# DylanAuty/ObjCAViT

Measured on AMD Instinct MI355X. Metric: images/sec (640x480, bs=16) forward depth inference, 3 batches of 16 in flight per GPU; AbsRel vs CPU ref, higher is better.
Workload: dtype f32 (fp16 / bf16 split contractions)

## Files before the change

### include/objcavit_hip.h

```cpp
#ifndef OBJCAVIT_HIP_H
#define OBJCAVIT_HIP_H

#include <stddef.h>
#include <stdint.h>

#ifdef __cplusplus
extern "C" {
#endif

typedef void* ocv_stream_t;

#define OCV_ABI_VERSION 5
int ocv_abi_version(void);
const char* ocv_last_error(void);

int ocv_range_flag_set(unsigned* flag);
int ocv_range_flag_take_fwd(unsigned* flag, unsigned* out, ocv_stream_t stream);
int ocv_attention_set_fp32_range(int on);
int ocv_attention_set_dispatch(int form);

#define OCV_ACT_NONE 0
#define OCV_ACT_RELU 1
#define OCV_ACT_LEAKY_RELU 2
#define OCV_ACT_SILU 3
// ... 92 lines not shown
                              void* workspace, size_t workspace_bytes, ocv_stream_t stream);

int ocv_pixel_dot_fwd(const float* feat, int channels_last, const float* queries, long q_bs, int q_ld, float* ram,
                      int B, int C, int Q, int P, ocv_stream_t stream);

size_t ocv_bin_head_workspace_bytes(int B, int n_bins, int C);
int ocv_bin_head_fold_fwd(const float* queries, long q_bs, int q_ld, const float* Wout, float* Wf, int B, int C, int Q,
                          int n_bins, ocv_stream_t stream);
int ocv_bin_head_folded_fwd(const float* feat, int channels_last, const float* Wf, const float* bout,
                            const float* centers, float* depth, int B, int C, int n_bins, int P, ocv_stream_t stream);
size_t ocv_bin_head_partials_bytes(int B, int P);
int ocv_bin_head_folded_ws_fwd(const float* feat, int channels_last, const float* Wf, const float* bout, const float* centers,
                               float* depth, int B, int C, int n_bins, int P, void* partials, size_t partials_bytes,
                               ocv_stream_t stream);
int ocv_bin_head_fwd(const float* feat, int channels_last, const float* queries, long q_bs, int q_ld, const float* Wout,
                     const float* bout, const float* centers, float* depth, int B, int C, int Q, int n_bins, int P,
                     void* workspace, size_t workspace_bytes, ocv_stream_t stream);
size_t ocv_bin_head_stats_partials_bytes(int B, int P);
int ocv_bin_head_folded_stats_fwd(const float* feat, int channels_last, const float* Wf, const float* bout, const float* centers,
                                  float* depth, int B, int C, int n_bins, int P, void* partials, size_t partials_bytes, float* var,
                                  float* pmax, ocv_stream_t stream);

int ocv_conv3x3_few_channels_fwd(const float* x, long stride_b, long stride_c, long stride_y, long stride_x, const float* w_taps,
                                 float* y, int B, int C, int H, int W, int Cout, ocv_stream_t stream);

int ocv_depthwise_conv_fwd(const float* in, const float* w, const float* bias, float* out, int B, int C, int H, int W,
                           int k, int stride, int pad_t, int pad_l, int Ho, int Wo, int act, ocv_stream_t stream);

int ocv_pointwise_conv_nhwc_fwd(const float* x, const float* gate, int rows_per_image, const float* W,
                                const float* bias, const float* residual, float* y, long M, int Cin, int Cout, int act,
                                ocv_stream_t stream);

size_t ocv_pointwise_packed_weight_elems(int Cin, int Cout);
int ocv_pointwise_split_set_dispatch(int family, int a, int b);
int ocv_pointwise_conv_nhwc_split_fwd(const float* x, const float* gate, int rows_per_image, const void* w_packed,
                                      const float* bias, const float* residual, float* y, long M, int Cin, int Cout,
                                      int act, ocv_stream_t stream);
int ocv_pointwise_conv_nhwc_split_hl_fwd(const float* x, const float* gate, int rows_per_image, const void* w_packed,
                                         const float* bias, const float* residual, float* y, void* y_hl, long M, int Cin,
                                         int Cout, int act, ocv_stream_t stream);
size_t ocv_pointwise_split_workspace_bytes(long M, int Cin, int Cout);
int ocv_pointwise_conv_nhwc_split_ws_fwd(const float* x, const float* gate, int rows_per_image, const void* w_packed,
                                         const float* bias, const float* residual, float* y, void* y_hl, long M, int Cin, int Cout,
                                         int act, void* workspace, size_t workspace_bytes, ocv_stream_t stream);
int ocv_pointwise_hl_set_dispatch(int rt, int tn);
int ocv_pointwise_hl_fwd(const void* x_hl, int Cin, const void* w_packed, long w_image_elems, int rows_per_image,
                         const float* bias, const float* residual, float* y, void* y_hl, long M, int Cout, int act,
                         ocv_stream_t stream);
int ocv_stem_conv_fwd(const float* x, const float* w, const float* bias, float* y, int B, int Cin, int H, int W, int Cout,
                      int k, int stride, int pad_t, int pad_l, int Ho, int Wo, int act, ocv_stream_t stream);
int ocv_depthwise_conv_nhwc_fwd(const float* in, const float* w, const float* bias, float* out, int B, int C, int H,
                                int W, int k, int stride, int pad_t, int pad_l, int Ho, int Wo, int act,
                                ocv_stream_t stream);
int ocv_depthwise_sum_tiles(int B, int C, int Ho, int Wo, int k, int stride);
int ocv_depthwise_conv_nhwc_sum_fwd(const float* in, const float* w, const float* bias, float* out, float* part, int B,
                                    int C, int H, int W, int k, int stride, int pad_t, int pad_l, int Ho, int Wo,
                                    ocv_stream_t stream);
int ocv_se_gate_partials_fwd(const float* part, int tiles, long pixels_per_image, const float* w1, const float* b1,
                             const float* w2t, const float* b2, float* gate, float* hidden_ws, int B, int C, int R,
                             ocv_stream_t stream);
int ocv_depthwise_conv_nhwc_sum_hl_fwd(const float* in, const float* w, const float* bias, float* out, void* out_hl, float* part,
                                       int B, int C, int H, int W, int k, int stride, int pad_t, int pad_l, int Ho, int Wo,
                                       ocv_stream_t stream);
int ocv_se_gate_weights_fwd(const float* part, int tiles, long pixels_per_image, const float* w1, const float* b1,
                            const float* w2t, const float* b2, const float* W, void* w_packed, long w_image_elems, float* gate,
                            float* hidden_ws, int B, int C, int R, int N, ocv_stream_t stream);


size_t ocv_channel_mean_workspace_bytes(int B, int C, long P);
int ocv_channel_mean_nhwc_fwd(const float* x, float* out, int B, int C, long P, void* workspace, size_t workspace_bytes,
                              ocv_stream_t stream);

int ocv_se_gate_fwd(const float* mean, const float* w1, const float* b1, const float* w2t, const float* b2, float* gate,
                    float* hidden_ws, int B, int C, int R, ocv_stream_t stream);

int ocv_conv_nhwc_fwd(const float* x1, int C1, const float* x2, int C2, const void* w_hi, const void* w_lo,
                      const float* bias, const float* residual, float* y, int B, int H, int W, int Cout, int ksize,
                      int act, ocv_stream_t stream);
int ocv_conv_nhwc_exact_fwd(const float* x1, int C1, const float* x2, int C2, const float* w_tap_major, const float* bias,
                            const float* residual, float* y, int B, int H, int W, int Cout, int ksize, int act,
                            ocv_stream_t stream);
int ocv_conv3x3_nhwc_strided_fwd(const float* x, int Cin, const void* w_hi, const void* w_lo, const float* bias,
                                 const float* residual, float* y, int B, int H, int W, int Cout, int stride, int pad_t,
                                 int pad_l, int Ho, int Wo, int act, ocv_stream_t stream);

int ocv_mbconv_expand_dw_tiles(int Ho, int Wo, int k, int stride);
int ocv_mbconv_expand_dw_fwd(const float* x, const void* w_packed, const float* bias_expand, const float* w_dw,
                             const float* bias_dw, float* y, float* part, int B, int H, int W, int Cin, int mid, int k,
                             int stride, int pad_t, int pad_l, int Ho, int Wo, ocv_stream_t stream);

size_t ocv_split_act_elems(int B, int H, int W, int C);

int ocv_conv_nhwc_split_fwd(const void* x_hl, int Cin, const void* w_hi, const void* w_lo, const float* bias,
                            const float* residual, float* y, void* y_hl, int B, int H, int W, int Cout, int ksize,
                            int act, ocv_stream_t stream);
size_t ocv_conv_nhwc_split_workspace_bytes(int B, int H, int W, int Cin, int Cout, int ksize);
int ocv_conv_nhwc_split_ws_fwd(const void* x_hl, int Cin, const void* w_hi, const void* w_lo, const float* bias,
                               const float* residual, float* y, void* y_hl, int B, int H, int W, int Cout, int ksize,
                               int act, void* workspace, size_t workspace_bytes, ocv_stream_t stream);
int ocv_conv_nhwc_split_x_fwd(const void* x_hl, int Cin, const void* w_hi, const void* w_lo, const float* oscale, int f16,
                              const float* bias, const float* residual, float* y, void* y_hl, int B, int H, int W, int Cout,
                              int ksize, int act, void* workspace, size_t workspace_bytes, ocv_stream_t stream);

int ocv_conv3x3_packed_taps_k(int Cin);
int ocv_conv3x3_split_packed_taps_fwd(const void* x_hl, int Cin, const void* w_hi, const void* w_lo, const float* oscale, int f16,
                                      const float* bias, const float* residual, float* y, void* y_hl, int B, int H, int W, int Cout,
// ... 84 lines not shown
```

### objcavit_amd/_lib.py

```python
from __future__ import annotations

import ctypes as C
import os
from typing import Optional

_HERE = os.path.dirname(os.path.abspath(__file__))
LIB_PATH = os.environ.get("OCV_LIB_PATH") or os.path.join(_HERE, "lib", "libobjcavit_hip.so")

_f32p = C.c_void_p
_u8p = C.c_void_p
_stream = C.c_void_p
ABI_VERSION = 5


class EncoderLayerParams(C.Structure):
    _fields_ = [("struct_size", C.c_size_t)] + [(n, C.c_void_p) for n in (
        "in_proj_w", "in_proj_b", "out_proj_w", "out_proj_b", "norm1_w", "norm1_b",
        "linear1_w", "linear1_b", "linear2_w", "linear2_b", "norm2_w", "norm2_b",
        "in_proj_p3", "out_proj_p3", "linear1_p3", "linear2_p3",
        "in_proj_h2", "out_proj_h2", "linear1_h2", "linear2_h2")]

    def __init__(self, *a, **kw):
        super().__init__(*a, **kw)
        self.struct_size = C.sizeof(EncoderLayerParams)
# ... 27 lines not shown
    "ocv_ffn_residual_layernorm_fwd": (C.c_int, [_f32p] * 7 + [C.c_float, _u8p, _f32p, C.c_int, C.c_int, C.c_int, _stream]),
    "ocv_split3_packed_elems": (C.c_size_t, [C.c_int, C.c_int]),
    "ocv_pack_split3_fwd": (C.c_int, [_f32p, C.c_int, C.c_int, C.c_int, C.c_void_p, _stream]),
    "ocv_linear_split3_fwd": (C.c_int, [_f32p, C.c_int, C.c_void_p, _f32p, _f32p, C.c_int, C.c_int, C.c_int, C.c_int, C.c_int, _stream]),
    "ocv_linear_residual_layernorm_split3_fwd": (C.c_int, [_f32p, C.c_int, C.c_void_p, _f32p, _f32p, C.c_int, _f32p, _f32p, C.c_float,
                                                           _u8p, _f32p, C.c_int, C.c_int, C.c_int, C.c_int, _stream]),
    "ocv_ffn_split3_workspace_bytes": (C.c_size_t, [C.c_int, C.c_int]),
    "ocv_ffn_residual_layernorm_split3_fwd": (C.c_int, [_f32p, C.c_void_p, _f32p, C.c_void_p, _f32p, _f32p, _f32p, C.c_float, _u8p, _f32p,
                                                        C.c_int, C.c_int, C.c_int, C.c_void_p, C.c_size_t, _stream]),
    "ocv_layer_tail_split3_fwd": (C.c_int, [_f32p, _f32p, C.POINTER(EncoderLayerParams), C.c_void_p, _f32p, C.c_float, _u8p, _f32p, _f32p,
                                            C.c_int, C.c_int, C.c_int, _stream]),
    "ocv_layer_tail_h2_fwd": (C.c_int, [_f32p, _f32p, C.POINTER(EncoderLayerParams), C.c_void_p, _f32p, C.c_float, _u8p, _f32p, _f32p,
                                            C.c_int, C.c_int, C.c_int, _stream]),
    "ocv_layer_tail_h2_groups": (C.c_int, [C.c_int, C.c_int]),
    "ocv_layer_tail_h2_workspace_bytes": (C.c_size_t, [C.c_int, C.c_int]),
    "ocv_layer_tail_h2_ws_fwd": (C.c_int, [_f32p, _f32p, C.POINTER(EncoderLayerParams), C.c_void_p, _f32p, C.c_float, _u8p, _f32p, _f32p,
                                           C.c_int, C.c_int, C.c_int, C.c_void_p, C.c_size_t, _stream]),
    "ocv_encoder_stack_workspace_bytes": (C.c_size_t, [C.c_int, C.c_int, C.c_int]),
    "ocv_encoder_stack_fwd": (C.c_int, [_f32p, C.POINTER(EncoderLayerParams), C.c_int, _u8p, C.c_int, _f32p, C.c_int, C.c_int, C.c_int,
                                        C.c_int, C.c_int, C.c_float, C.c_void_p, C.c_size_t, _stream]),
    "ocv_encoder_layer_workspace_bytes": (C.c_size_t, [C.c_int, C.c_int, C.c_int, C.c_int]),
    "ocv_encoder_layer_fwd": (C.c_int, [_f32p, C.POINTER(EncoderLayerParams), _u8p, C.c_int, _f32p, C.c_int, C.c_int,
                                        C.c_int, C.c_int, C.c_int, C.c_float, C.c_void_p, C.c_size_t, _stream]),
    "ocv_pointwise_conv_nhwc_split_hl_fwd": (C.c_int, [_f32p, _f32p, C.c_int, C.c_void_p, _f32p, _f32p, _f32p, C.c_void_p, C.c_long, C.c_int,
                                                       C.c_int, C.c_int, _stream]),
    "ocv_pointwise_split_workspace_bytes": (C.c_size_t, [C.c_long, C.c_int, C.c_int]),
    "ocv_pointwise_conv_nhwc_split_ws_fwd": (C.c_int, [_f32p, _f32p, C.c_int, C.c_void_p, _f32p, _f32p, _f32p, C.c_void_p, C.c_long, C.c_int,
                                                       C.c_int, C.c_int, C.c_void_p, C.c_size_t, _stream]),
    "ocv_pointwise_hl_set_dispatch": (C.c_int, [C.c_int, C.c_int]),
    "ocv_pointwise_hl_fwd": (C.c_int, [C.c_void_p, C.c_int, C.c_void_p, C.c_long, C.c_int, _f32p, _f32p, _f32p, C.c_void_p, C.c_long,
                                       C.c_int, C.c_int, _stream]),
    "ocv_depthwise_conv_nhwc_sum_hl_fwd": (C.c_int, [_f32p, _f32p, _f32p, _f32p, C.c_void_p, _f32p] + [C.c_int] * 10 + [_stream]),
    "ocv_se_gate_weights_fwd": (C.c_int, [_f32p, C.c_int, C.c_long, _f32p, _f32p, _f32p, _f32p, _f32p, C.c_void_p, C.c_long, _f32p,
                                          _f32p, C.c_int, C.c_int, C.c_int, C.c_int, _stream]),
    "ocv_patch_embed_workspace_bytes": (C.c_size_t, [C.c_int, C.c_int, C.c_int, C.c_int, C.c_int]),
    "ocv_patch_embed_split_workspace_bytes": (C.c_size_t, [C.c_int, C.c_int, C.c_int, C.c_int, C.c_int]),
    "ocv_patch_embed_split_fwd": (C.c_int, [C.c_void_p, C.c_int, C.c_void_p, C.c_void_p, _f32p, C.c_int, _f32p, _f32p, C.c_long, _f32p, C.c_int,
                                            C.c_int, C.c_int, C.c_int, C.c_void_p, C.c_size_t, _stream]),
    "ocv_patch_embed_fwd": (C.c_int, [_f32p, C.c_int, _f32p, _f32p, _f32p, C.c_long, _f32p, C.c_int, C.c_int, C.c_int, C.c_int,
                                      C.c_int, C.c_void_p, C.c_size_t, _stream]),
    "ocv_pixel_dot_fwd": (C.c_int, [_f32p, C.c_int, _f32p, C.c_long, C.c_int, _f32p, C.c_int, C.c_int, C.c_int, C.c_int, _stream]),
    "ocv_bin_head_workspace_bytes": (C.c_size_t, [C.c_int, C.c_int, C.c_int]),
    "ocv_bin_head_fold_fwd": (C.c_int, [_f32p, C.c_long, C.c_int, _f32p, _f32p, C.c_int, C.c_int, C.c_int, C.c_int, _stream]),
    "ocv_bin_head_folded_fwd": (C.c_int, [_f32p, C.c_int, _f32p, _f32p, _f32p, _f32p, C.c_int, C.c_int, C.c_int, C.c_int, _stream]),
    "ocv_bin_head_partials_bytes": (C.c_size_t, [C.c_int, C.c_int]),
    "ocv_bin_head_folded_ws_fwd": (C.c_int, [_f32p, C.c_int, _f32p, _f32p, _f32p, _f32p, C.c_int, C.c_int, C.c_int, C.c_int,
                                             C.c_void_p, C.c_size_t, _stream]),
    "ocv_bin_head_stats_partials_bytes": (C.c_size_t, [C.c_int, C.c_int]),
    "ocv_bin_head_folded_stats_fwd": (C.c_int, [_f32p, C.c_int, _f32p, _f32p, _f32p, _f32p, C.c_int, C.c_int, C.c_int, C.c_int,
                                                C.c_void_p, C.c_size_t, _f32p, _f32p, _stream]),
    "ocv_bin_head_fwd": (C.c_int, [_f32p, C.c_int, _f32p, C.c_long, C.c_int, _f32p, _f32p, _f32p, _f32p, C.c_int, C.c_int,
                                   C.c_int, C.c_int, C.c_int, C.c_void_p, C.c_size_t, _stream]),
    "ocv_depthwise_conv_fwd": (C.c_int, [_f32p, _f32p, _f32p, _f32p] + [C.c_int] * 11 + [_stream]),
    "ocv_depthwise_sum_tiles": (C.c_int, [C.c_int] * 6),
    "ocv_depthwise_conv_nhwc_sum_fwd": (C.c_int, [_f32p] * 5 + [C.c_int] * 10 + [_stream]),
    "ocv_se_gate_partials_fwd": (C.c_int, [_f32p, C.c_int, C.c_long, _f32p, _f32p, _f32p, _f32p, _f32p, _f32p, C.c_int,
                                           C.c_int, C.c_int, _stream]),
    "ocv_depth_metrics_workspace_bytes": (C.c_size_t, [C.c_int] * 3),
    "ocv_depth_metrics_fwd": (C.c_int, [_f32p, _f32p, C.c_int, C.c_int, _f32p, C.c_int, C.c_int, C.c_float, C.c_float] + [C.c_int] * 4 +
                              [C.c_long, _f32p, C.c_int, C.c_void_p, C.c_size_t, _stream]),
    "ocv_depth_metrics_loss_workspace_bytes": (C.c_size_t, [C.c_int] * 4),
    "ocv_depth_metrics_loss_fwd": (C.c_int, [_f32p, _f32p, C.c_int, C.c_int, _f32p, C.c_int, C.c_int, C.c_float, C.c_float] + [C.c_int] * 4 +
                                   [_f32p, C.c_int, C.c_long, _f32p, _f32p, C.c_int, C.c_void_p, C.c_size_t, _stream]),
    "ocv_frame_ingest_fwd": (C.c_int, [_u8p, C.c_long, C.c_long, C.c_int, C.c_int, C.c_int, C.c_int, _f32p, _f32p, C.c_int, C.c_int, C.c_int,
                                       C.c_int, C.c_long, _stream]),
    "ocv_depth_ingest_fwd": (C.c_int, [C.c_void_p, C.c_long, C.c_long, C.c_int, C.c_int, C.c_int, C.c_int, C.c_float, _f32p, C.c_int, C.c_int,
                                       C.c_int, _stream]),
    "ocv_depth_finalize_fwd": (C.c_int, [_f32p, _f32p, C.c_int, C.c_int, C.c_float, C.c_float, C.c_int, C.c_int, _f32p, C.c_void_p, C.c_float,
                                         _u8p, _u8p, C.c_float, C.c_float, C.c_int, _stream]),
    "ocv_depth_finalize_stats_fwd": (C.c_int, [_f32p] * 6 + [C.c_int, C.c_int, C.c_float, C.c_float, C.c_int, C.c_int, _f32p, _f32p, C.c_int,
                                               _stream]),
    "ocv_object_depth_fwd": (C.c_int, [_f32p, _f32p, _f32p, C.c_long, C.c_void_p, C.c_int, C.c_int, C.c_int, C.c_int, C.c_float,
                                       C.POINTER(C.c_double), C.c_int, _f32p, _stream]),
    "ocv_object_metrics_workspace_bytes": (C.c_size_t, [C.c_int] * 3),
    "ocv_object_metrics_fwd": (C.c_int, [_f32p, _f32p, C.c_int, C.c_int, _f32p, C.c_int, C.c_int, C.c_float, C.c_float] + [C.c_int] * 4 +
                               [_f32p, C.c_long, C.c_void_p, C.c_int, C.c_int, C.c_float, _f32p, _f32p, C.c_void_p, C.c_size_t, _stream]),
    "ocv_depth_unproject_workspace_bytes": (C.c_size_t, [C.c_int] * 5),
    "ocv_depth_unproject_fwd": (C.c_int, [_f32p, _f32p, _f32p, _f32p, _u8p, C.c_long, C.c_long] + [C.c_int] * 9 + [C.c_float] * 4 +
                                [C.c_int, _f32p, C.c_void_p, C.c_void_p, C.c_void_p, C.c_void_p, C.c_size_t, _stream]),
    "ocv_conv3x3_few_channels_fwd": (C.c_int, [_f32p, C.c_long, C.c_long, C.c_long, C.c_long, _f32p, _f32p] + [C.c_int] * 5 + [_stream]),
    "ocv_stem_conv_fwd": (C.c_int, [_f32p, _f32p, _f32p, _f32p] + [C.c_int] * 12 + [_stream]),
    "ocv_pointwise_packed_weight_elems": (C.c_size_t, [C.c_int, C.c_int]),
    "ocv_pointwise_split_set_dispatch": (C.c_int, [C.c_int, C.c_int, C.c_int]),
    "ocv_pointwise_conv_nhwc_split_fwd": (C.c_int, [_f32p, _f32p, C.c_int, C.c_void_p, _f32p, _f32p, _f32p,
                                                    C.c_long, C.c_int, C.c_int, C.c_int, C.c_void_p]),
    "ocv_pointwise_conv_nhwc_fwd": (C.c_int, [_f32p, _f32p, C.c_int, _f32p, _f32p, _f32p, _f32p, C.c_long, C.c_int, C.c_int,
                                              C.c_int, _stream]),
    "ocv_depthwise_conv_nhwc_fwd": (C.c_int, [_f32p, _f32p, _f32p, _f32p] + [C.c_int] * 11 + [_stream]),
    "ocv_channel_mean_workspace_bytes": (C.c_size_t, [C.c_int, C.c_int, C.c_long]),
    "ocv_channel_mean_nhwc_fwd": (C.c_int, [_f32p, _f32p, C.c_int, C.c_int, C.c_long, C.c_void_p, C.c_size_t, _stream]),
    "ocv_se_gate_fwd": (C.c_int, [_f32p] * 7 + [C.c_int] * 3 + [_stream]),
    "ocv_conv_nhwc_fwd": (C.c_int, [_f32p, C.c_int, _f32p, C.c_int, C.c_void_p, C.c_void_p, _f32p, _f32p, _f32p] +
                          [C.c_int] * 6 + [_stream]),
    "ocv_conv3x3_nhwc_strided_fwd": (C.c_int, [_f32p, C.c_int, C.c_void_p, C.c_void_p, _f32p, _f32p, _f32p] + [C.c_int] * 10 + [_stream]),
    "ocv_conv_nhwc_exact_fwd": (C.c_int, [_f32p, C.c_int, _f32p, C.c_int, _f32p, _f32p, _f32p, _f32p] + [C.c_int] * 6 + [_stream]),
    "ocv_mbconv_expand_dw_tiles": (C.c_int, [C.c_int] * 4),
    "ocv_mbconv_expand_dw_fwd": (C.c_int, [_f32p, C.c_void_p, _f32p, _f32p, _f32p, _f32p, _f32p] + [C.c_int] * 11 + [_stream]),
    "ocv_regressor_bins_fwd": (C.c_int, [_f32p, C.c_long, _f32p, _f32p, _f32p, _f32p, _f32p, _f32p, C.c_int, C.c_int, C.c_int, C.c_int, C.c_float,
                                         C.c_int, C.c_float, C.c_float, _f32p, _f32p, _f32p, C.c_int, _stream]),
    "ocv_bin_edges_fwd": (C.c_int, [_f32p, C.c_int, C.c_float, C.c_float, _f32p, _f32p, _f32p, C.c_int, C.c_int, _stream]),
    "ocv_object_tokens_pad_fwd": (C.c_int, [_f32p, C.c_void_p, C.c_float, _f32p, _u8p, C.c_int, C.c_int, C.c_int, _stream]),
    "ocv_object_front_pad_fwd": (C.c_int, [_f32p, C.c_void_p, C.c_int, C.c_int, C.c_float, _f32p, _u8p] + [C.c_int] * 4 + [_stream]),
    "ocv_split_act_elems": (C.c_size_t, [C.c_int] * 4),
    "ocv_conv_nhwc_split_fwd": (C.c_int, [C.c_void_p, C.c_int, C.c_void_p, C.c_void_p, _f32p, _f32p, _f32p, C.c_void_p]
                                + [C.c_int] * 6 + [_stream]),
    "ocv_conv_nhwc_split_workspace_bytes": (C.c_size_t, [C.c_int] * 6),
# ... 62 lines not shown
```

### objcavit_amd/csrc/depthwise_se.hip

```cpp
#include <stdlib.h>

#include "common.hpp"
#include "../../include/objcavit_hip.h"

namespace {

typedef __bf16 dw_bf16x4 __attribute__((ext_vector_type(4)));

struct DWSArgs {
  const float *in, *w, *bias;
  float *out, *part;
  __bf16* out_hl;
  int C, H, W, Ho, Wo, pad_t, pad_l;
  int QL, PL, RY;
  int wox, nwork, tiles, chunks;
};

template <int K, int S, int PX>
__global__ __launch_bounds__(256, 2) void dw_slide_kernel(DWSArgs p) {
  constexpr int NIN = (PX - 1) * S + K;
  constexpr bool WLDS = K > 3;
  __shared__ float4 red[256];
  __shared__ float4 wsh[WLDS ? K * K * 64 : 1];
  const int tid = threadIdx.x;
// ... 93 lines not shown
              r4.x = fast_silu(r4.x); r4.y = fast_silu(r4.y); r4.z = fast_silu(r4.z); r4.w = fast_silu(r4.w);
              if (p.out != nullptr) *reinterpret_cast<float4*>(ob + (roff + o) * p.C) = r4;
              if (p.out_hl != nullptr) {
                const float f[4] = {r4.x, r4.y, r4.z, r4.w};
                dw_bf16x4 h, l;
#pragma unroll
                for (int e = 0; e < 4; ++e) {
                  const __bf16 hb = (__bf16)f[e];
                  h[e] = hb;
                  l[e] = (__bf16)(f[e] - (float)hb);
                }
                __bf16* d = ohb + (roff + o) * 2 * p.C;
                *reinterpret_cast<dw_bf16x4*>(d) = h;
                *reinterpret_cast<dw_bf16x4*>(d + 32) = l;
              }
              sum.x += r4.x; sum.y += r4.y; sum.z += r4.z; sum.w += r4.w;
            }
          }
        }
      }
    }
  }
  red[tid] = sum;
  __syncthreads();
  if (pl == 0 && cq < c4n) {
    float4 t = red[q];
    for (int l = 1; l < p.PL; ++l) {
      const float4 u = red[l * p.QL + q];
      t.x += u.x; t.y += u.y; t.z += u.z; t.w += u.w;
    }
    float* dst = p.part + ((b * p.tiles + tile) * (long)p.C) + c;
    *reinterpret_cast<float4*>(dst) = t;
  }
}

struct DWSGeom { int QL, PL, RY, PX, chunks, wox, nruns, nwork, tiles; };
DWSGeom dws_geom(int B, int C, int Ho, int Wo, int k, int stride) {
  DWSGeom g;
  g.PX = (stride == 1 && k == 3) ? 4 : ((stride == 2 && k == 5) ? 1 : 2);
  const int c4n = C / 4;
  g.chunks = (c4n + 63) / 64;
  g.QL = (c4n + g.chunks - 1) / g.chunks;
  g.PL = 256 / g.QL;
  g.wox = (Wo + g.PX - 1) / g.PX;
  int ry = 8;
  while (ry > 2 && (long)g.wox * ((Ho + ry - 1) / ry) * g.chunks * B < 800L * g.PL) ry >>= 1;
  g.RY = ry;
  g.nruns = (Ho + ry - 1) / ry;
  g.nwork = g.wox * g.nruns;
  g.tiles = (g.nwork + g.PL - 1) / g.PL;
  return g;
}

__global__ __launch_bounds__(1024) void se_hidden_partials_kernel(const float* __restrict__ part, int tiles, float inv,
                                                                 const float* __restrict__ w1, const float* __restrict__ b1,
                                                                 float* __restrict__ hid, int C, int R) {
  extern __shared__ float sm[];
  float* mean = sm;
  float* red = sm + C;
  const int tid = threadIdx.x, lane = tid & 63, wave = tid >> 6;
  const long b = blockIdx.y;
  const float* pb = part + b * tiles * (long)C;
  const int nq = C >> 2;
  const int TG = nq >= 1024 ? 1 : min(tiles, 1024 / nq);
  for (int idx = tid; idx < TG * nq; idx += 1024) {
    const int q = idx % nq, tg = idx / nq;
    float4 a[8];
#pragma unroll
    for (int j = 0; j < 8; ++j) a[j] = make_float4(0.f, 0.f, 0.f, 0.f);
    const float* src = pb + 4 * q;
    for (int t0 = tg; t0 < tiles; t0 += 8 * TG) {
      float4 u[8];
#pragma unroll
      for (int j = 0; j < 8; ++j) u[j] = ld4(src + (long)min(t0 + j * TG, tiles - 1) * C);
#pragma unroll
      for (int j = 0; j < 8; ++j) {
        const bool ok = t0 + j * TG < tiles;
        a[j].x += ok ? u[j].x : 0.f; a[j].y += ok ? u[j].y : 0.f; a[j].z += ok ? u[j].z : 0.f; a[j].w += ok ? u[j].w : 0.f;
      }
    }
    float4 r;
    r.x = ((a[0].x + a[1].x) + (a[2].x + a[3].x)) + ((a[4].x + a[5].x) + (a[6].x + a[7].x));
    r.y = ((a[0].y + a[1].y) + (a[2].y + a[3].y)) + ((a[4].y + a[5].y) + (a[6].y + a[7].y));
    r.z = ((a[0].z + a[1].z) + (a[2].z + a[3].z)) + ((a[4].z + a[5].z) + (a[6].z + a[7].z));
    r.w = ((a[0].w + a[1].w) + (a[2].w + a[3].w)) + ((a[4].w + a[5].w) + (a[6].w + a[7].w));
    *reinterpret_cast<float4*>(red + tg * C + 4 * q) = r;
  }
  __syncthreads();
  for (int c = tid; c < C; c += 1024) {
    float s = red[c];
    for (int tg = 1; tg < TG; ++tg) s += red[tg * C + c];
    mean[c] = s * inv;
  }
  __syncthreads();
  const int r = blockIdx.x * 16 + wave;
  if (r >= R) return;
  const float* wr = w1 + (long)r * C;
  float s0 = 0.f, s1 = 0.f, s2 = 0.f, s3 = 0.f;
  int q = lane;
  for (; q + 192 < nq; q += 256) {
    const float4 u0 = ld4(wr + 4 * q), u1 = ld4(wr + 4 * (q + 64)), u2 = ld4(wr + 4 * (q + 128)), u3 = ld4(wr + 4 * (q + 192));
    const float4 m0 = *reinterpret_cast<const float4*>(mean + 4 * q), m1 = *reinterpret_cast<const float4*>(mean + 4 * (q + 64));
    const float4 m2 = *reinterpret_cast<const float4*>(mean + 4 * (q + 128)), m3 = *reinterpret_cast<const float4*>(mean + 4 * (q + 192));
    s0 = fmaf(u0.x, m0.x, fmaf(u0.y, m0.y, fmaf(u0.z, m0.z, fmaf(u0.w, m0.w, s0))));
    s1 = fmaf(u1.x, m1.x, fmaf(u1.y, m1.y, fmaf(u1.z, m1.z, fmaf(u1.w, m1.w, s1))));
    s2 = fmaf(u2.x, m2.x, fmaf(u2.y, m2.y, fmaf(u2.z, m2.z, fmaf(u2.w, m2.w, s2))));
// ... 168 lines not shown
        s0 = fmaf(w[(long)r * C], hs[r], s0);
        s1 = fmaf(w[(long)(r + 1) * C], hs[r + 1], s1);
        s2 = fmaf(w[(long)(r + 2) * C], hs[r + 2], s2);
        s3 = fmaf(w[(long)(r + 3) * C], hs[r + 3], s3);
      }
      for (; r < R; ++r) s0 = fmaf(w[(long)r * C], hs[r], s0);
      g = fast_sigmoid((s0 + s1) + (s2 + s3));
      if (gate != nullptr) gate[b * C + c] = g;
    }
    gs[tid] = g;
  }
  __syncthreads();
  const int o = tid >> 5, nl = tid & 31;
  const int k = k0 + 8 * o;
  const int Kp = (C + 15) & ~15;
  if (k >= Kp) return;
  const int nsteps = Kp >> 4, s = k >> 4, hh = (k >> 3) & 1;
  float g8[8];
#pragma unroll
  for (int e = 0; e < 8; ++e) g8[e] = gs[8 * o + e];
  __bf16* ob = wpk + b * img_elems;
  const int ntl = (N + 31) >> 5;
  for (int jt = 0; jt < ntl; ++jt) {
    const int n = jt * 32 + nl;
    float f[8];
#pragma unroll
    for (int e = 0; e < 8; ++e) f[e] = 0.f;
    if (n < N && k < C) {
      const float4 u = ld4(W + (long)n * C + k), v = ld4(W + (long)n * C + k + 4);
      f[0] = u.x * g8[0]; f[1] = u.y * g8[1]; f[2] = u.z * g8[2]; f[3] = u.w * g8[3];
      f[4] = v.x * g8[4]; f[5] = v.y * g8[5]; f[6] = v.z * g8[6]; f[7] = v.w * g8[7];
    }
    typedef __bf16 bf16x8_t __attribute__((ext_vector_type(8)));
    bf16x8_t h, l;
#pragma unroll
    for (int e = 0; e < 8; ++e) {
      const __bf16 hb = (__bf16)f[e];
      h[e] = hb;
      l[e] = (__bf16)(f[e] - (float)hb);
    }
    __bf16* d = ob + (((long)jt * nsteps + s) * 2) * 512 + (hh * 32 + nl) * 8;
    *reinterpret_cast<bf16x8_t*>(d) = h;
    *reinterpret_cast<bf16x8_t*>(d + 512) = l;
  }
}

template <int K, int S, int PX>
int launch_dws(const DWSArgs& a, const DWSGeom& g, int B, hipStream_t st) {
  hipLaunchKernelGGL((dw_slide_kernel<K, S, PX>), dim3((unsigned)((long)g.tiles * g.chunks * B)), dim3(256), 0, st, a);
  OCV_CHECK_LAUNCH("ocv_depthwise_conv_nhwc_sum_fwd");
  return 0;
}

}

extern "C" int ocv_depthwise_sum_tiles(int B, int C, int Ho, int Wo, int k, int stride) {
  if (B < 1 || C < 4 || C % 4 != 0 || Ho < 1 || Wo < 1 || (k != 3 && k != 5) || (stride != 1 && stride != 2)) return 0;
  return dws_geom(B, C, Ho, Wo, k, stride).tiles;
}

extern "C" int ocv_depthwise_conv_nhwc_sum_fwd(const float* in, const float* w, const float* bias, float* out, float* part,
                                               int B, int C, int H, int W, int k, int stride, int pad_t, int pad_l,
                                               int Ho, int Wo, ocv_stream_t stream) {
  return ocv_depthwise_conv_nhwc_sum_hl_fwd(in, w, bias, out, nullptr, part, B, C, H, W, k, stride, pad_t, pad_l, Ho, Wo, stream);
}

namespace {
int dws_run(const float* in, const float* w, const float* bias, float* out, void* out_hl, float* part,
            int B, int C, int H, int W, int k, int stride, int pad_t, int pad_l, int Ho, int Wo, ocv_stream_t stream) {
  OCV_CHECK_ARG(in && w && (out || out_hl) && part, "ocv_depthwise_conv_nhwc_sum_fwd: null pointer");
  OCV_CHECK_ARG(out_hl == nullptr || (C % 32 == 0 && ocv_aligned16(out_hl)), "ocv_depthwise_conv_nhwc_sum_hl_fwd: the split output needs C to be a multiple of 32 (got %d) and 16-byte alignment", C);
  OCV_CHECK_ARG(B >= 1 && C >= 4 && C % 4 == 0 && H >= 1 && W >= 1 && Ho >= 1 && Wo >= 1, "ocv_depthwise_conv_nhwc_sum_fwd: bad sizes (C must be a multiple of 4)");
  OCV_CHECK_ARG((k == 3 || k == 5) && (stride == 1 || stride == 2), "ocv_depthwise_conv_nhwc_sum_fwd: k must be 3 or 5 and stride 1 or 2");
  OCV_CHECK_ARG(pad_t >= 0 && pad_l >= 0 && pad_t < k && pad_l < k, "ocv_depthwise_conv_nhwc_sum_fwd: bad padding");
  OCV_CHECK_ARG((Ho - 1) * stride - pad_t < H && (Wo - 1) * stride - pad_l < W, "ocv_depthwise_conv_nhwc_sum_fwd: output larger than the padded input allows");
  OCV_CHECK_ARG(ocv_aligned16(in) && ocv_aligned16(w) && ocv_aligned16(out) && ocv_aligned16(bias) && ocv_aligned16(part), "ocv_depthwise_conv_nhwc_sum_fwd: operands must be 16-byte aligned");
  const DWSGeom g = dws_geom(B, C, Ho, Wo, k, stride);
  OCV_CHECK_ARG((long)g.tiles * g.chunks * B < (1L << 31), "ocv_depthwise_conv_nhwc_sum_fwd: too many workgroups");
  DWSArgs a{in, w, bias, out, part, (__bf16*)out_hl, C, H, W, Ho, Wo, pad_t, pad_l, g.QL, g.PL, g.RY, g.wox, g.nwork, g.tiles, g.chunks};
  hipStream_t st = (hipStream_t)stream;
  if (k == 3 && stride == 1) return launch_dws<3, 1, 4>(a, g, B, st);
  if (k == 3 && stride == 2) return launch_dws<3, 2, 2>(a, g, B, st);
  if (k == 5 && stride == 1) return launch_dws<5, 1, 2>(a, g, B, st);
  return launch_dws<5, 2, 1>(a, g, B, st);
}
}

extern "C" int ocv_depthwise_conv_nhwc_sum_hl_fwd(const float* in, const float* w, const float* bias, float* out, void* out_hl,
                                                  float* part, int B, int C, int H, int W, int k, int stride, int pad_t,
                                                  int pad_l, int Ho, int Wo, ocv_stream_t stream) {
  return dws_run(in, w, bias, out, out_hl, part, B, C, H, W, k, stride, pad_t, pad_l, Ho, Wo, stream);
}

extern "C" int ocv_se_gate_partials_fwd(const float* part, int tiles, long pixels_per_image, const float* w1,
                                        const float* b1, const float* w2t, const float* b2, float* gate, float* hidden_ws,
                                        int B, int C, int R, ocv_stream_t stream) {
  OCV_CHECK_ARG(part && w1 && b1 && w2t && b2 && gate && hidden_ws, "ocv_se_gate_partials_fwd: null pointer");
  OCV_CHECK_ARG(B >= 1 && B <= 65535 && C >= 1 && R >= 1 && R <= 256 && tiles >= 1 && pixels_per_image >= 1, "ocv_se_gate_partials_fwd: bad sizes (R <= 256)");
  OCV_CHECK_ARG(C <= 8192 && C % 4 == 0, "ocv_se_gate_partials_fwd: C must be a multiple of 4, at most 8192 (got %d)", C);
  hipStream_t st = (hipStream_t)stream;
  const size_t lds = (size_t)(C + (C >= 4096 ? C : 4096)) * sizeof(float);
  constexpr int max_c = 1536, max_r = 64;
  if (C <= max_c && R <= max_r && R <= 128) {
    hipLaunchKernelGGL(se_fused_small_kernel, dim3((C + 255) / 256, B), dim3(1024), lds + 128 * sizeof(float), st, part, tiles,
                       1.0f / (float)pixels_per_image, w1, b1, w2t, b2, gate, C, R);
    OCV_CHECK_LAUNCH("ocv_se_gate_partials_fwd(fused)");
    return 0;
  }
  hipLaunchKernelGGL(se_hidden_partials_kernel, dim3((R + 15) / 16, B), dim3(1024), lds, st, part, tiles,
                     1.0f / (float)pixels_per_image, w1, b1, hidden_ws, C, R);
  OCV_CHECK_LAUNCH("ocv_se_gate_partials_fwd(hidden)");
  hipLaunchKernelGGL(se_gate_hid_kernel, dim3((C + 255) / 256, B), dim3(256), 0, st, (const float*)hidden_ws, w2t, b2, gate, C, R);
  OCV_CHECK_LAUNCH("ocv_se_gate_partials_fwd(gate)");
  return 0;
}

extern "C" int ocv_se_gate_weights_fwd(const float* part, int tiles, long pixels_per_image, const float* w1, const float* b1,
                                       const float* w2t, const float* b2, const float* W, void* w_packed, long w_image_elems,
                                       float* gate, float* hidden_ws, int B, int C, int R, int N, ocv_stream_t stream) {
  OCV_CHECK_ARG(part && w1 && b1 && w2t && b2 && W && w_packed && hidden_ws, "ocv_se_gate_weights_fwd: null pointer");
  OCV_CHECK_ARG(B >= 1 && B <= 65535 && C >= 8 && C % 8 == 0 && R >= 1 && R <= 256 && N >= 1 && tiles >= 1 && pixels_per_image >= 1,
                "ocv_se_gate_weights_fwd: bad sizes (C a multiple of 8, R <= 256)");
  OCV_CHECK_ARG(C <= 8192, "ocv_se_gate_weights_fwd: C too large (%d)", C);
  OCV_CHECK_ARG(w_image_elems >= (long)ocv_pointwise_packed_weight_elems(C, N) && (w_image_elems & 7) == 0 && ocv_aligned16(w_packed) && ocv_aligned16(W),
                "ocv_se_gate_weights_fwd: w_image_elems must hold one packed matrix (ocv_pointwise_packed_weight_elems) and keep 16-byte alignment");
  hipStream_t st = (hipStream_t)stream;
  const size_t lds = (size_t)(C + (C >= 4096 ? C : 4096)) * sizeof(float);
  hipLaunchKernelGGL(se_hidden_partials_kernel, dim3((R + 15) / 16, B), dim3(1024), lds, st, part, tiles,
                     1.0f / (float)pixels_per_image, w1, b1, hidden_ws, C, R);
  OCV_CHECK_LAUNCH("ocv_se_gate_weights_fwd(hidden)");
  const int Kp = (C + 15) / 16 * 16;
  hipLaunchKernelGGL(se_gate_weights_kernel, dim3((Kp + 63) / 64, B), dim3(256), 0, st, (const float*)hidden_ws, w2t, b2, W,
                     (__bf16*)w_packed, w_image_elems, gate, C, R, N);
// ... 4 lines not shown
```

Before: 1105.

## Add LDS row-ring depthwise 5x5 kernel with async global-to-LDS producer wave

Adds a new 5x5 depthwise conv+SiLU+SE-partial kernel. One producer wave streams input rows into an LDS ring buffer with global_load_lds and counted vmcnt waits, while consumer waves compute output rows from LDS. It also adds XCD-aware workgroup remapping and a new tile geometry. It is dispatched by default for k=5 layers (stride 1, or stride 2 with large outputs) and is meant to replace redundant register-window global loads with reused, prefetched rows. The risks are lower occupancy from the large LDS footprint and barrier overhead on every row.

```diff
diff --git a/include/objcavit_hip.h b/include/objcavit_hip.h
--- a/include/objcavit_hip.h
+++ b/include/objcavit_hip.h
@@ -168,6 +168,7 @@
 int ocv_depthwise_conv_nhwc_fwd(const float* in, const float* w, const float* bias, float* out, int B, int C, int H,
                                 int W, int k, int stride, int pad_t, int pad_l, int Ho, int Wo, int act,
                                 ocv_stream_t stream);
+int ocv_depthwise_set_dispatch(int mode);
 int ocv_depthwise_sum_tiles(int B, int C, int Ho, int Wo, int k, int stride);
 int ocv_depthwise_conv_nhwc_sum_fwd(const float* in, const float* w, const float* bias, float* out, float* part, int B,
                                     int C, int H, int W, int k, int stride, int pad_t, int pad_l, int Ho, int Wo,
diff --git a/objcavit_amd/_lib.py b/objcavit_amd/_lib.py
--- a/objcavit_amd/_lib.py
+++ b/objcavit_amd/_lib.py
@@ -103,6 +103,7 @@
     "ocv_bin_head_fwd": (C.c_int, [_f32p, C.c_int, _f32p, C.c_long, C.c_int, _f32p, _f32p, _f32p, _f32p, C.c_int, C.c_int,
                                    C.c_int, C.c_int, C.c_int, C.c_void_p, C.c_size_t, _stream]),
     "ocv_depthwise_conv_fwd": (C.c_int, [_f32p, _f32p, _f32p, _f32p] + [C.c_int] * 11 + [_stream]),
+    "ocv_depthwise_set_dispatch": (C.c_int, [C.c_int]),
     "ocv_depthwise_sum_tiles": (C.c_int, [C.c_int] * 6),
     "ocv_depthwise_conv_nhwc_sum_fwd": (C.c_int, [_f32p] * 5 + [C.c_int] * 10 + [_stream]),
     "ocv_se_gate_partials_fwd": (C.c_int, [_f32p, C.c_int, C.c_long, _f32p, _f32p, _f32p, _f32p, _f32p, _f32p, C.c_int,
diff --git a/objcavit_amd/csrc/depthwise_se.hip b/objcavit_amd/csrc/depthwise_se.hip
--- a/objcavit_amd/csrc/depthwise_se.hip
+++ b/objcavit_amd/csrc/depthwise_se.hip
@@ -169,6 +169,226 @@
   return g;
 }
 
+__device__ __attribute__((aligned(256))) float ocv_dw_zero_page[64];
+
+typedef __attribute__((address_space(1))) const void* dwr_gptr;
+typedef __attribute__((address_space(3))) void* dwr_lptr;
+
+struct DWRArgs {
+  const float *in, *w, *bias;
+  float *out, *part;
+  __bf16* out_hl;
+  int C, H, W, Ho, Wo, pad_t, pad_l;
+  int QL, TH;
+  int nxt, tiles, chunks;
+};
+
+constexpr int dwr_threads(int s) { return s == 1 ? 256 : 320; }
+constexpr int dwr_waves_per_simd(int s) { return s == 1 ? 2 : 3; }
+
+template <int S, int QLP>
+struct DWRShape {
+  static constexpr int K = 5, PX = S == 1 ? 2 : 1;
+  static constexpr int NCT = dwr_threads(S) - 64;
+  static constexpr int PL = NCT / QLP, TW = PX * PL;
+  static constexpr int RW = S * TW + K - S;
+  static constexpr int NI = (RW * QLP + 63) / 64;
+  static constexpr int ROWE = NI * 64;
+  static constexpr int NB = S == 1 ? (QLP == 32 ? 9 : 10) : (QLP == 32 ? 7 : 8);
+  static constexpr size_t LDS = ((size_t)NB * ROWE + NCT) * sizeof(float4);
+  static_assert(2 * LDS <= 160 * 1024, "two workgroups per CU");
+};
+
+template <int S, int QLP>
+__global__ __launch_bounds__(dwr_threads(S), dwr_waves_per_simd(S)) void dw_rows_kernel(DWRArgs p) {
+  using G = DWRShape<S, QLP>;
+  constexpr int K = G::K, PX = G::PX, PL = G::PL, NCT = G::NCT, TW = G::TW, RW = G::RW, NI = G::NI, ROWE = G::ROWE, NB = G::NB;
+  constexpr int NIN = (PX - 1) * S + K;
+  constexpr int AHEAD = NB - S - K;
+  static_assert(NCT % QLP == 0 && 64 % QLP == 0 && AHEAD >= 0 && AHEAD * NI <= 63, "counted vmcnt must fit its 6-bit field");
+  extern __shared__ __attribute__((aligned(16))) float4 dwr_sm[];
+  float4* ring = dwr_sm;
+  float4* red = dwr_sm + NB * ROWE;
+  const int tid = threadIdx.x;
+  const int c4n = p.C >> 2;
+  int tile, chunk;
+  long b;
+  {
+    const int nwg = gridDim.x;
+    int wg = blockIdx.x;
+    const int qq = nwg >> 3, r = nwg & 7, xcd = wg & 7, idx = wg >> 3;
+    wg = (xcd < r ? xcd * (qq + 1) : r * (qq + 1) + (xcd - r) * qq) + idx;
+    tile = wg % p.tiles;
+    const int rest = wg / p.tiles;
+    chunk = rest % p.chunks;
+    b = rest / p.chunks;
+  }
+  const int band = tile / p.nxt, xt = tile - band * p.nxt;
+  const int y0 = band * p.TH, y1 = min(p.Ho, y0 + p.TH);
+  const int iyb = y0 * S - p.pad_t;
+  const int ixb = xt * TW * S - p.pad_l;
+
+  if (tid >= NCT) {
+    const int lane = tid & 63;
+    const int qd = lane % QLP, cq = chunk * p.QL + qd;
+    const bool qok = qd < p.QL && cq < c4n;
+    int coff[NI];
+#pragma unroll
+    for (int j = 0; j < NI; ++j) {
+      const int px = j * (64 / QLP) + lane / QLP, ix = ixb + px;
+      coff[j] = qok && px < RW && ix >= 0 && ix < p.W ? ix * p.C + cq * 4 : -1;
+    }
+    const float* ib = p.in + b * (long)p.H * p.W * p.C;
+    const int nrel = (y1 - y0 - 1) * S + K;
+    auto issue = [&](int rel, int slot) {
+      const int iy = iyb + rel;
+      const bool rok = rel < nrel && iy >= 0 && iy < p.H;
+      const float* row = ib + (long)(rok ? iy : 0) * p.W * p.C;
+      __attribute__((address_space(3))) float4* dst = (__attribute__((address_space(3))) float4*)ring + slot * ROWE;
+#pragma unroll
+      for (int j = 0; j < NI; ++j) {
+        const float* src = rok && coff[j] >= 0 ? row + coff[j] : ocv_dw_zero_page;
+        __builtin_amdgcn_global_load_lds((dwr_gptr)src, (dwr_lptr)(dst + j * 64), 16, 0, 0);
+      }
+    };
+#pragma unroll
+    for (int rel = 0; rel < NB - S; ++rel) issue(rel, rel);
+    int slot = NB - S, rel = NB - S;
+#pragma unroll 1
+    for (int y = y0; y < y1; ++y) {
+      asm volatile("s_waitcnt vmcnt(%0)" ::"n"(AHEAD * NI) : "memory");
+      __builtin_amdgcn_s_barrier();
+#pragma unroll
+      for (int sidx = 0; sidx < S; ++sidx) {
+        issue(rel, slot);
+        ++rel;
+        slot = slot + 1 == NB ? 0 : slot + 1;
+      }
+    }
+    asm volatile("s_waitcnt vmcnt(0)" ::: "memory");
+  } else {
+    const int q = tid % QLP, pl = tid / QLP;
+    const int cq = chunk * p.QL + q;
+    const bool active = q < p.QL && cq < c4n;
+    const int c = (active ? cq : 0) * 4;
+    const int ox = (xt * PL + pl) * PX;
+    const bool act0 = active && ox < p.Wo;
+    const bool ok1 = PX > 1 && ox + 1 < p.Wo;
+    float4 wv[K * K];
+#pragma unroll
+    for (int t = 0; t < K * K; ++t) wv[t] = ld4(p.w + (long)t * p.C + c);
+    const float4 bv = p.bias ? ld4(p.bias + c) : make_float4(0.f, 0.f, 0.f, 0.f);
+    float4 sum = make_float4(0.f, 0.f, 0.f, 0.f);
+    const long opix = (b * p.Ho + y0) * (long)p.Wo + ox;
+    float* ob = p.out + opix * p.C + c;
+    __bf16* ohb = p.out_hl + opix * 2 * p.C + (c >> 5) * 64 + (c & 31);
+    const float4* rp = ring + pl * PX * S * QLP + q;
+    int s0 = 0;
+#pragma unroll 1
+    for (int y = y0; y < y1; ++y) {
+      asm volatile("s_waitcnt lgkmcnt(0)" ::: "memory");
+      __builtin_amdgcn_s_barrier();
+      asm volatile("" ::: "memory");
+      if (act0) {
+        float4 acc[PX];
+#pragma unroll
+        for (int o = 0; o < PX; ++o) acc[o] = bv;
+#pragma unroll
+        for (int r = 0; r < K; ++r) {
+          __builtin_amdgcn_sched_barrier(0);
+          const int t = s0 + r;
+          const float4* rr = rp + (t >= NB ? t - NB : t) * ROWE;
+          float4 x[NIN];
+#pragma unroll
+          for (int j = 0; j < NIN; ++j) x[j] = rr[j * QLP];
+#pragma unroll
+          for (int j = 0; j < K; ++j) {
+            const float4 w4 = wv[r * K + j];
+#pragma unroll
+            for (int o = 0; o < PX; ++o) {
+              acc[o].x = fmaf(w4.x, x[o * S + j].x, acc[o].x); acc[o].y = fmaf(w4.y, x[o * S + j].y, acc[o].y);
+              acc[o].z = fmaf(w4.z, x[o * S + j].z, acc[o].z); acc[o].w = fmaf(w4.w, x[o * S + j].w, acc[o].w);
+            }
+          }
+        }
+        const long roff = (long)(y - y0) * p.Wo;
+#pragma unroll
+        for (int o = 0; o < PX; ++o) {
+          const bool ok = o == 0 || ok1;
+          const int oo = ok ? o : 0;
+          float4 r4 = acc[o];
+          r4.x = fast_silu(r4.x); r4.y = fast_silu(r4.y); r4.z = fast_silu(r4.z); r4.w = fast_silu(r4.w);
+          if (o > 0) {
+            float4 f4 = acc[0];
+            f4.x = fast_silu(f4.x); f4.y = fast_silu(f4.y); f4.z = fast_silu(f4.z); f4.w = fast_silu(f4.w);
+            r4.x = ok ? r4.x : f4.x; r4.y = ok ? r4.y : f4.y; r4.z = ok ? r4.z : f4.z; r4.w = ok ? r4.w : f4.w;
+          }
+          if (p.out != nullptr) *reinterpret_cast<float4*>(ob + (roff + oo) * p.C) = r4;
+          if (p.out_hl != nullptr) {
+            const float f[4] = {r4.x, r4.y, r4.z, r4.w};
+            dw_bf16x4 h, l;
+#pragma unroll
+            for (int e = 0; e < 4; ++e) {
+              const __bf16 hb = (__bf16)f[e];
+              h[e] = hb;
+              l[e] = (__bf16)(f[e] - (float)hb);
+            }
+            __bf16* d = ohb + (roff + oo) * 2 * p.C;
+            *reinterpret_cast<dw_bf16x4*>(d) = h;
+            *reinterpret_cast<dw_bf16x4*>(d + 32) = l;
+          }
+          sum.x += ok ? r4.x : 0.f; sum.y += ok ? r4.y : 0.f; sum.z += ok ? r4.z : 0.f; sum.w += ok ? r4.w : 0.f;
+        }
+      }
+      s0 = s0 + S >= NB ? s0 + S - NB : s0 + S;
+    }
+    red[tid] = sum;
+  }
+  __syncthreads();
+  if (tid < QLP && tid < p.QL && chunk * p.QL + tid < c4n) {
+    float4 t = red[tid];
+    for (int l = 1; l < PL; ++l) {
+      const float4 u = red[l * QLP + tid];
+      t.x += u.x; t.y += u.y; t.z += u.z; t.w += u.w;
+    }
+    float* dst = p.part + ((b * p.tiles + tile) * (long)p.C) + (chunk * p.QL + tid) * 4;
+    *reinterpret_cast<float4*>(dst) = t;
+  }
+}
+
+struct DWRGeom { int QLP, QL, chunks, nxt, TH, tiles; };
+DWRGeom dwr_geom(int B, int C, int Ho, int Wo, int stride) {
+  DWRGeom g{};
+  const int c4n = C / 4, px = stride == 1 ? 2 : 1;
+  double best = -1.0;
+  for (int qlp = 32; qlp >= 16; qlp >>= 1) {
+    const int chunks = (c4n + qlp - 1) / qlp, tw = px * (stride == 1 ? 192 : 256) / qlp, nxt = (Wo + tw - 1) / tw;
+    const double eff = (double)c4n / ((double)chunks * qlp) * Wo / ((double)nxt * tw) * (stride * tw) / (stride * tw + 5 - stride);
+    if (eff > best * 1.0000001) {
+      best = eff;
+      g.QLP = qlp;
+      g.chunks = chunks;
+      g.nxt = nxt;
+    }
+  }
+  g.QL = (c4n + g.chunks - 1) / g.chunks;
+  int nb = 1;
+  while ((long)B * g.chunks * g.nxt * nb < 1024 && (Ho + nb) / (nb + 1) >= 8) ++nb;
+  g.TH = (Ho + nb - 1) / nb;
+  g.tiles = g.nxt * ((Ho + g.TH - 1) / g.TH);
+  return g;
+}
+
+int& dw_dispatch() {
+  static int mode = 0;
+  return mode;
+}
+bool dw_use_rows(int C, int Ho, int Wo, int k, int stride) {
+  const int mode = dw_dispatch();
+  if (mode == 1 || k != 5 || ((long)stride * Wo + k) * C >= (1L << 30)) return false;
+  return mode == 2 || stride == 1 || (long)Ho * Wo >= 1200;
+}
+
 __global__ __launch_bounds__(1024) void se_hidden_partials_kernel(const float* __restrict__ part, int tiles, float inv,
                                                                  const float* __restrict__ w1, const float* __restrict__ b1,
                                                                  float* __restrict__ hid, int C, int R) {
@@ -443,10 +663,30 @@
   return 0;
 }
 
+template <int S, int QLP>
+int launch_dwr(const DWRArgs& a, int B, hipStream_t st) {
+  static bool attr = false;
+  if (!attr) {
+    (void)hipFuncSetAttribute((const void*)dw_rows_kernel<S, QLP>, hipFuncAttributeMaxDynamicSharedMemorySize, 160 * 1024);
+    attr = true;
+  }
+  constexpr size_t lds = DWRShape<S, QLP>::LDS;
+  hipLaunchKernelGGL((dw_rows_kernel<S, QLP>), dim3((unsigned)((long)a.tiles * a.chunks * B)), dim3(dwr_threads(S)), lds, st, a);
+  OCV_CHECK_LAUNCH("ocv_depthwise_conv_nhwc_sum_fwd(rows)");
+  return 0;
+}
+
+}
+
+extern "C" int ocv_depthwise_set_dispatch(int mode) {
+  OCV_CHECK_ARG(mode >= 0 && mode <= 2, "ocv_depthwise_set_dispatch: mode must be 0 (automatic), 1 (register window) or 2 (LDS rows), got %d", mode);
+  dw_dispatch() = mode;
+  return 0;
 }
 
 extern "C" int ocv_depthwise_sum_tiles(int B, int C, int Ho, int Wo, int k, int stride) {
   if (B < 1 || C < 4 || C % 4 != 0 || Ho < 1 || Wo < 1 || (k != 3 && k != 5) || (stride != 1 && stride != 2)) return 0;
+  if (dw_use_rows(C, Ho, Wo, k, stride)) return dwr_geom(B, C, Ho, Wo, stride).tiles;
   return dws_geom(B, C, Ho, Wo, k, stride).tiles;
 }
 
@@ -466,10 +706,18 @@
   OCV_CHECK_ARG(pad_t >= 0 && pad_l >= 0 && pad_t < k && pad_l < k, "ocv_depthwise_conv_nhwc_sum_fwd: bad padding");
   OCV_CHECK_ARG((Ho - 1) * stride - pad_t < H && (Wo - 1) * stride - pad_l < W, "ocv_depthwise_conv_nhwc_sum_fwd: output larger than the padded input allows");
   OCV_CHECK_ARG(ocv_aligned16(in) && ocv_aligned16(w) && ocv_aligned16(out) && ocv_aligned16(bias) && ocv_aligned16(part), "ocv_depthwise_conv_nhwc_sum_fwd: operands must be 16-byte aligned");
+  hipStream_t st = (hipStream_t)stream;
+  if (dw_use_rows(C, Ho, Wo, k, stride)) {
+    const DWRGeom r = dwr_geom(B, C, Ho, Wo, stride);
+    OCV_CHECK_ARG((long)r.tiles * r.chunks * B < (1L << 31), "ocv_depthwise_conv_nhwc_sum_fwd: too many workgroups");
+    OCV_CHECK_ARG((long)W * C < (1L << 31), "ocv_depthwise_conv_nhwc_sum_fwd: input rows of 2^31 elements or more");
+    DWRArgs a{in, w, bias, out, part, (__bf16*)out_hl, C, H, W, Ho, Wo, pad_t, pad_l, r.QL, r.TH, r.nxt, r.tiles, r.chunks};
+    if (stride == 1) return r.QLP == 32 ? launch_dwr<1, 32>(a, B, st) : launch_dwr<1, 16>(a, B, st);
+    return r.QLP == 32 ? launch_dwr<2, 32>(a, B, st) : launch_dwr<2, 16>(a, B, st);
+  }
   const DWSGeom g = dws_geom(B, C, Ho, Wo, k, stride);
   OCV_CHECK_ARG((long)g.tiles * g.chunks * B < (1L << 31), "ocv_depthwise_conv_nhwc_sum_fwd: too many workgroups");
   DWSArgs a{in, w, bias, out, part, (__bf16*)out_hl, C, H, W, Ho, Wo, pad_t, pad_l, g.QL, g.PL, g.RY, g.wox, g.nwork, g.tiles, g.chunks};
-  hipStream_t st = (hipStream_t)stream;
   if (k == 3 && stride == 1) return launch_dws<3, 1, 4>(a, g, B, st);
   if (k == 3 && stride == 2) return launch_dws<3, 2, 2>(a, g, B, st);
   if (k == 5 && stride == 1) return launch_dws<5, 1, 2>(a, g, B, st);
```

Result: faster. 1123, median of 6 (+1.6%).
